# marcin119a/vae-los-angeles

Measured on AMD Instinct MI355X. Metric: training samples/sec, MultiModalVAE batch 65536, higher is better.
Workload: dtype bf16

## Files before the change

### include/mmvae_hip.h

```cpp
#ifndef MMVAE_HIP_H
#define MMVAE_HIP_H
#include <stdint.h>

#ifdef __cplusplus
extern "C" {
#endif

#define MMVAE_OK 0
#define MMVAE_ERR_ARG (-1)
#define MMVAE_ERR_DTYPE (-2)

enum { MMVAE_F32 = 0, MMVAE_BF16 = 1 };
enum { MMVAE_PREC_F32 = 0, MMVAE_PREC_BF16 = 1 };
enum { MMVAE_PRO_NONE = 0, MMVAE_PRO_BN_RELU_DROP = 1, MMVAE_PRO_BN_BWD_APPLY = 2 };
enum { MMVAE_EPI_STORE = 0, MMVAE_EPI_RELU_MASK = 1, MMVAE_EPI_BN_BWD = 2, MMVAE_EPI_LOSS_MSE = 3, MMVAE_EPI_LOSS_BCE_LOGIT = 4 };
enum { MMVAE_ACT_NONE = 0, MMVAE_ACT_RELU = 1, MMVAE_ACT_SIGMOID = 2 };

#define MMVAE_TILE 128

int mmvae_abi_version(void);
int mmvae_set_tuning(int32_t key, int32_t value);

typedef struct {
    const float* src; void* dst;
// ... 98 lines not shown
    const float* scale; const float* shift;
    const uint8_t* mask; int64_t ld_mask; float inv_keep;
    const void* finalize;
    const void* w; int64_t ldw; const float* bias;
} mmvae_latent_enc;
typedef struct {
    int32_t prec, B, L, n_mod;
    mmvae_latent_enc enc_a, enc_b;
    const float* table; const int64_t* site; int32_t S;
    const float* eps;
    float* mu; float* logvar;
    void* z; int64_t ldz;
    const void* w_stem; int64_t ldw_stem; const float* bias_stem; int32_t N_stem;
    void* h0; int64_t ldh0;
} mmvae_latent_fwd_args;
int mmvae_latent_fwd(const mmvae_latent_fwd_args* args, void* stream);

typedef struct {
    int32_t prec, B, S, L, hidden;
    const void* h0; int64_t ldh0;
    const void* w; int64_t ldw; const void* wt; int64_t ldwt; const float* bias;
    const int64_t* site; const float* class_weights;
    const float* mu; const float* logvar;
    float beta, gamma; const float* beta_gamma_dev;
    double* sums;
    float* g_c; int64_t ld_gc;
    void* d0; int64_t ldd0;
    float* g_mu; float* g_lv;
} mmvae_class_tail_args;
int mmvae_class_tail(const mmvae_class_tail_args* args, void* stream);
int mmvae_class_tail_fits(int32_t prec, int32_t S, int32_t hidden, int32_t L, int64_t ldh0, int64_t ldd0);

typedef struct {
    int32_t B, A, D, S, L;
    const float* recon_a; const void* a; int64_t ld_ra, ld_a;
    const float* recon_b; const void* b; int64_t ld_rb, ld_b;
    const float* logits; int64_t ld_logits; const int64_t* site; const float* class_weights;
    const float* mu; const float* logvar;
    float beta, gamma;
    double* sums;
    void* g_a; int32_t g_a_dtype; int64_t ld_ga;
    void* g_b; int32_t g_b_dtype; int64_t ld_gb; int32_t grad_b_wrt_logit;
    float* g_c; int64_t ld_gc;
    float* g_mu; float* g_lv;
    const float* beta_gamma_dev;
    int32_t a_dtype, b_dtype;
} mmvae_loss_args;
int mmvae_vae_loss(const mmvae_loss_args* args, void* stream);
int mmvae_loss_finalize(const double* sums, float beta, float gamma, const float* beta_gamma_dev, float* out5, void* stream);

int mmvae_sigmoid_bwd(int32_t M, int32_t N, const float* g, int64_t ldg, const float* p, int64_t ldpp,
                      void* out, int32_t out_dtype, int64_t ldo, void* stream);

int mmvae_scale_if_needed(void* x, int32_t dtype, int64_t n, const float* scale_dev, void* stream);
#define MMVAE_SCALE_MAX 8
typedef struct { void* x; int64_t n; int32_t dtype; int32_t pad_; } mmvae_scale_item;
int mmvae_scale_many(const mmvae_scale_item* items_host, int32_t n_items, const float* scale_dev, void* stream);

#define MMVAE_CTR_COPIES 16384
int mmvae_noise(uint8_t* mask, int64_t n_mask, float keep_prob, float* eps, int64_t n_eps, uint64_t seed, uint64_t offset,
                uint64_t* offset_dev, int32_t advance, void* stream);
int mmvae_counter_add(uint64_t* counter_dev, uint64_t inc, void* stream);

#define MMVAE_GATHER_MAX 4
typedef struct { const void* src; void* dst; int64_t src_row_stride; int64_t dst_row_stride; int32_t row_bytes; int32_t pad_; } mmvae_gather_item;
int mmvae_gather_rows(const mmvae_gather_item* items_host, int32_t n_items, const int64_t* idx_dev, int32_t rows,
// ... 118 lines not shown
```

### vae-los-angeles_amd/csrc/common.h

```cpp
#pragma once
#include <hip/hip_runtime.h>
#include <stdint.h>
#include "mmvae_hip.h"

namespace mm {

typedef __bf16 bf16;
typedef __attribute__((ext_vector_type(8))) __bf16 bf16x8;
typedef __attribute__((ext_vector_type(4))) __bf16 bf16x4;
typedef __attribute__((ext_vector_type(2))) __bf16 bf16x2;
typedef __attribute__((ext_vector_type(4))) float f32x4;
typedef __attribute__((ext_vector_type(2))) float f32x2;
typedef __attribute__((ext_vector_type(4))) short s16x4;

constexpr int WAVE = 64;
constexpr int TILE = 128;
constexpr int NTHREADS = 256;
constexpr int ROW_BYTES = 128;
constexpr int NUM_CU = 256;

template <typename CT> struct Mma;

template <> struct Mma<bf16> {
    static constexpr int EPC = 8;
// ... 109 lines not shown
    if (n < 0 || n > STAMP_SLOTS) return MMVAE_ERR_ARG;
    hipError_t e = hipMemcpyFromSymbol(out, sym, n * sizeof(uint64_t));
    if (e != hipSuccess || !reset) return (int)e;
    const uint64_t z[STAMP_SLOTS] = {};
    return (int)hipMemcpyToSymbol(sym, z, sizeof(z));
}
int stamp_read_nt(uint64_t*, int, int);
int stamp_read_nt2(uint64_t*, int, int);
int stamp_read_ntp(uint64_t*, int, int);
int stamp_read_tn(uint64_t*, int, int);
int stamp_read_tnw(uint64_t*, int, int);
#else
#define STAMP_T(x)
#define STAMP_ADD(i, d)
#define STAMP_ONLY(...)
#define UNSTAMPED(...) __VA_ARGS__
#define STAMP_BUFFER(name)
#define STAMP_ENTRY()
#endif


struct Tuning {
    int nt_wide_min_m = NUM_CU * 128;
    int nt2_on = 1;
    long split_bytes = 1L << 32;
    long block_bytes = 1L << 31;
    int tn_wide_on = 1;
    int bnbwd_stream = 1;
    int relu_stream = 1;
    int ntp_on = 1;
    int ntp_min_m = 16384;
    int latent_on = 1;
    int class_tail_on = 1;
};
inline Tuning g_tuning;

constexpr int NOT_TAKEN = 1 << 30;

template <auto Kernel, typename... Args>
inline int launch_lds(dim3 grid, dim3 block, int lds, hipStream_t st, const Args&... args) {
    static bool attr_done = false;
    if (!attr_done) {
        hipError_t e = hipFuncSetAttribute((const void*)Kernel, hipFuncAttributeMaxDynamicSharedMemorySize, lds);
        if (e != hipSuccess) return (int)e;
        attr_done = true;
    }
    hipLaunchKernelGGL(Kernel, grid, block, lds, st, args...);
    return (int)hipGetLastError();
}

inline bool needs_row_blocks(long M, long row_bytes) { return M * row_bytes >= g_tuning.split_bytes; }

template <typename F>
inline int for_row_blocks(long M, long row_bytes, F&& block) {
    long rows = g_tuning.block_bytes / row_bytes;
    if (rows <= 0) return MMVAE_ERR_ARG;
    const long nblk = (M + rows - 1) / rows;
    long even = (M + nblk - 1) / nblk;
    if (even >= 256) even = (even + 255) & ~255L;
    if (even <= rows) rows = even;
    else if (rows >= 256) rows &= ~255L;
    for (long r0 = 0; r0 < M; r0 += rows) {
        const int rc = block(r0, (int)(M - r0 < rows ? M - r0 : rows));
        if (rc) return rc;
    }
    return 0;
// ... 31 lines not shown
```

### vae-los-angeles_amd/csrc/elementwise.hip

```cpp
#include <vector>
#include "common.h"
#include "mmvae_hip.h"
#include "fuse_math.h"
#include "loss_terms.h"

namespace mm {

__global__ __launch_bounds__(256) void prep_weights_kernel(const mmvae_prep_item* __restrict__ items) {
    const mmvae_prep_item it = items[blockIdx.y];
    __shared__ float tile[32][33];
    const int tx = threadIdx.x & 31, ty = threadIdx.x >> 5;
    const int tiles_c = (it.dst_cols + 31) / 32, tiles_r = (it.dst_rows + 31) / 32;
    auto put = [&](int r, int c, float v) {
        if (it.dst_dtype == MMVAE_BF16) ((bf16*)it.dst)[(long)r * it.dst_ld + c] = (bf16)v;
        else ((float*)it.dst)[(long)r * it.dst_ld + c] = v;
    };
    for (int t = blockIdx.x; t < tiles_r * tiles_c; t += gridDim.x) {
        const int tr = t / tiles_c, tc = t - tr * tiles_c;
        if (it.transpose) {
#pragma unroll
            for (int k = 0; k < 4; ++k) {
                const int sr = tc * 32 + ty + 8 * k, sc = tr * 32 + tx;
                tile[ty + 8 * k][tx] = (sr < it.src_rows && sc < it.src_cols) ? it.src[(long)sr * it.src_ld + sc] : 0.f;
            }
// ... 209 lines not shown
    }
}

__global__ __launch_bounds__(256) void fuse_bwd_kernel(mmvae_fuse_bwd_args a, int rows_per_block, int use_lds) {
    extern __shared__ float sT[];
    const int L2 = 2 * a.L;
    if (use_lds) { for (int i = threadIdx.x; i < a.S * L2; i += blockDim.x) sT[i] = 0.f; __syncthreads(); }
    const int b0 = blockIdx.x * rows_per_block, b1 = min(a.B, b0 + rows_per_block);
    float* dtab = a.d_table ? a.d_table + (long)(blockIdx.x % (a.table_copies > 0 ? a.table_copies : 1)) * a.S * L2 : nullptr;
    const float inv_n = 1.f / (float)a.n_mod;
    constexpr int U = 4;
    const long iend = (long)b1 * a.L;
    for (long i0 = (long)b0 * a.L + threadIdx.x; i0 < iend; i0 += (long)U * blockDim.x) {
        float dz[U], gm[U], gl[U], ep[U], lv[U];
        int bb[U], ll[U];
        long sidx[U];
#pragma unroll
        for (int u = 0; u < U; ++u) {
            const long i = min(i0 + (long)u * blockDim.x, iend - 1);
            const int b = (int)(i / a.L), l = (int)(i - (long)b * a.L);
            bb[u] = b; ll[u] = l;
            dz[u] = a.dz[(long)b * a.lddz + l];
            if (a.dz2) dz[u] += a.dz2[(long)b * a.lddz + l];
            if (a.dz3) dz[u] += a.dz3[(long)b * a.lddz + l];
            gm[u] = a.g_mu ? a.g_mu[i] : 0.f; gl[u] = a.g_lv ? a.g_lv[i] : 0.f;
            ep[u] = a.eps[i]; lv[u] = a.logvar[i];
            sidx[u] = a.d_table ? a.site[b] : 0;
            if (sidx[u] < 0 || sidx[u] >= a.S) sidx[u] = -1;
        }
#pragma unroll
        for (int u = 0; u < U; ++u) {
            if (i0 + (long)u * blockDim.x >= iend) break;
            const int b = bb[u], l = ll[u];
            float dmu = gm[u] + dz[u];
            float dlv = gl[u] + dz[u] * ep[u] * expf(0.5f * lv[u]) * 0.5f;
            if (a.n_mod > 1) { dmu *= inv_n; dlv *= inv_n; }
            a.d_heads[(long)b * a.ld_heads + l] = dmu;
            a.d_heads[(long)b * a.ld_heads + a.L + l] = dlv;
            if (a.d_heads_lp) {
                bf16* lp = (bf16*)a.d_heads_lp + (long)b * a.ld_heads_lp;
                lp[l] = (bf16)dmu; lp[a.L + l] = (bf16)dlv;
                if (l == 0) for (int e = 2 * a.L; e < a.ld_heads_lp; ++e) lp[e] = (bf16)0.f;
            }
            if (a.d_table && sidx[u] >= 0) {
                const long sx = sidx[u];
                if (use_lds) { atomicAdd(&sT[sx * L2 + l], dmu); atomicAdd(&sT[sx * L2 + a.L + l], dlv); }
                else { unsafeAtomicAdd(&dtab[sx * L2 + l], dmu); unsafeAtomicAdd(&dtab[sx * L2 + a.L + l], dlv); }
            }
        }
    }
    if (use_lds && a.d_table) {
        __syncthreads();
        for (int i = threadIdx.x; i < a.S * L2; i += blockDim.x) if (sT[i] != 0.f) unsafeAtomicAdd(&dtab[i], sT[i]);
    }
}

template <typename GT, int V>
__device__ __forceinline__ void store_vec(GT* p, const float* v) {
    GT o[V];
#pragma unroll
    for (int e = 0; e < V; ++e) o[e] = from_f32<GT>(v[e]);
    if constexpr (sizeof(GT) * V == 16) *(f32x4*)p = *(f32x4*)o;
    else if constexpr (sizeof(GT) * V == 8) *(f32x2*)p = *(f32x2*)o;
    else if constexpr (sizeof(GT) * V == 4) *(float*)p = *(float*)o;
    else for (int e = 0; e < V; ++e) p[e] = o[e];
}

struct RowWalk {
    unsigned cv, dc, vpr;
// ... 750 lines not shown
```

### vae-los-angeles_amd/csrc/fuse_math.h

```cpp
#pragma once
#include "common.h"

namespace mm {

__device__ __forceinline__ float fuse_reparam_elem(float& mu, float& lv, int n_mod, float inv_n, float eps) {
    if (n_mod > 1) { mu *= inv_n; lv *= inv_n; }
    return mu + eps * expf(0.5f * lv);
}

}
```

### vae-los-angeles_amd/csrc/gemm_nt.hip

```cpp
#include "common.h"
#include "mmvae_hip.h"
#include "gemm_src.h"
#include "gemm_nt_epi.h"
#include "gemm_nt2.h"

namespace mm {

STAMP_BUFFER(nt)

__device__ __forceinline__ int swz(int row, int chunk) { return row * ROW_BYTES + ((chunk ^ (row & 7)) << 4); }

template <int WN> struct NtLds {
    static constexpr int BUF = (TILE + 64 * WN) * ROW_BYTES;
    static constexpr int STAGE = 2 * BUF;
    static constexpr int ECOL = STAGE + 4096 + 4 * 64 * WN * 4;
    static constexpr int TOTAL = ECOL + 8 * 64 * WN * 4;
};

template <typename CT, typename Src, typename Epi, int WN>
__global__ __launch_bounds__(128 * WN, 2)
void gemm_nt_kernel(Src src, const CT* __restrict__ W, long ldw, int M, int N, int K, int gx, int gy, Epi epi)
{
    constexpr int EPC = Mma<CT>::EPC;
    constexpr int BK = ROW_BYTES / (int)sizeof(CT);
// ... 275 lines not shown
        SrcBnReluDrop<CT> s{(const CT*)a->a, a->lda, a->M, a->K, a->pro_scale, a->pro_shift, a->pro_mask, a->ld_pro_mask, a->pro_inv_keep, bn_fin_of(a)};
        return dispatch_epi<CT>(a, s, st);
    }
    if (a->a_dtype == MMVAE_BF16) {
        if constexpr (sizeof(CT) == 2) {
            if (a->lda % 8 || ((uintptr_t)a->a & 15)) return MMVAE_ERR_ARG;
            SrcPlain<CT, bf16, 8> s{(const bf16*)a->a, a->lda, a->M, a->K};
            return dispatch_epi<CT>(a, s, st);
        }
        return MMVAE_ERR_DTYPE;
    }
    return with_src_f32<CT>(a->a, a->lda, a->M, a->K, [&](const auto& s) { return dispatch_epi<CT>(a, s, st); });
}

}

extern "C" int mmvae_set_tuning(int32_t key, int32_t value) {
    mm::Tuning& t = mm::g_tuning;
    switch (key) {
    case 0: t.nt_wide_min_m = value; return 0;
    case 2: t.nt2_on = value; return 0;
    case 3:
        if (value != 0 && (value < 17 || value > 32)) return MMVAE_ERR_ARG;
        t.split_bytes = value ? 1L << value : mm::Tuning{}.split_bytes;
        t.block_bytes = t.split_bytes / 2;
        return 0;
    case 4: t.tn_wide_on = value; return 0;
    case 6: t.bnbwd_stream = value; return 0;
    case 7: t.relu_stream = value; return 0;
    case 8: t.ntp_on = value; return 0;
    case 9: t.ntp_min_m = value; return 0;
    case 10: t.latent_on = value; return 0;
    case 12: t.class_tail_on = value; return 0;
    }
    return MMVAE_ERR_ARG;
}

extern "C" int mmvae_gemm_nt(const mmvae_gemm_nt_args* a, void* stream) {
    if (!a || !a->a || !a->w || (!a->c && !(a->epilogue == MMVAE_EPI_BN_BWD && a->bn_phase == 0))) return MMVAE_ERR_ARG;
    if (a->M <= 0 || a->N <= 0 || a->K <= 0) return MMVAE_ERR_ARG;
    if (a->ldw % 64 || ((uintptr_t)a->w & 15)) return MMVAE_ERR_ARG;
    const long lim = 1L << 32;
    if (((long)a->N + 256) * a->ldw * 4 >= lim) return MMVAE_ERR_ARG;
    const long a_row = (long)a->lda * (a->a_dtype == MMVAE_BF16 ? 2 : 4);
    long row_bytes = a_row > (long)a->ld_pro_mask ? a_row : (long)a->ld_pro_mask;
    if (!mm::bn_fin_ok(a)) return MMVAE_ERR_ARG;
    if (mm::needs_row_blocks(a->M, row_bytes)) {
        if (a->pro_finalize || a->pro_out) return MMVAE_ERR_ARG;
        const bool loss_epi = a->epilogue == MMVAE_EPI_LOSS_MSE || a->epilogue == MMVAE_EPI_LOSS_BCE_LOGIT;
        const long hsz = loss_epi ? (a->h_dtype == MMVAE_BF16 ? 2 : 4) : (a->prec == MMVAE_PREC_BF16 ? 2 : 4);
        return mm::for_row_blocks(a->M, row_bytes, [&](long r0, int rows) {
            mmvae_gemm_nt_args s = *a;
            s.M = rows;
            s.a = (const char*)a->a + r0 * a_row;
            if (a->c) s.c = (char*)a->c + r0 * a->ldc * (a->c_dtype == MMVAE_BF16 ? 2 : 4);
            if (a->h) s.h = (const char*)a->h + r0 * a->ldh * hsz;
            if (a->pro_mask) s.pro_mask = a->pro_mask + r0 * a->ld_pro_mask;
            if (a->epi_mask) s.epi_mask = a->epi_mask + r0 * a->ld_epi_mask;
            return mmvae_gemm_nt(&s, stream);
        });
    }
    hipStream_t st = (hipStream_t)stream;
    { const int rc = mm::ntp_dispatch(a, st); if (rc != mm::NOT_TAKEN) return rc; }
    if (a->pro_out) return MMVAE_ERR_ARG;
    if (a->prec == MMVAE_PREC_BF16) return mm::dispatch_src<mm::bf16>(a, st);
    if (a->prec == MMVAE_PREC_F32) return mm::dispatch_src<float>(a, st);
// ... 5 lines not shown
```

### vae-los-angeles_amd/mmvae/_lib.py

```python
import ctypes as C
import os

_HERE = os.path.dirname(os.path.abspath(__file__))
LIB_PATH = os.environ.get("MMVAE_LIB_PATH") or os.path.join(_HERE, "libmmvae_hip.so")
ABI_VERSION = 20

F32, BF16 = 0, 1
PREC_F32, PREC_BF16 = 0, 1
PRO_NONE, PRO_BN_RELU_DROP, PRO_BN_BWD_APPLY = 0, 1, 2
TABLE_COPIES = 8
EPI_STORE, EPI_RELU_MASK, EPI_BN_BWD, EPI_LOSS_MSE, EPI_LOSS_BCE_LOGIT = 0, 1, 2, 3, 4
ACT_NONE, ACT_RELU, ACT_SIGMOID = 0, 1, 2
TILE = 128
TN_GROUP_MAX = 8
KNN_MAXK = 96
SIL_MAXC = 64
PCA_MAXK = 64
LN_MAXN = 1024
WCE_MAXC = 64
CTR_COPIES = 16384

i32, i64, f32, vp = C.c_int32, C.c_int64, C.c_float, C.c_void_p


# ... 52 lines not shown
                ("heads_a", vp), ("heads_b", vp), ("ld_heads", i64),
                ("table", vp), ("site", vp), ("S", i32),
                ("eps", vp), ("mu", vp), ("logvar", vp),
                ("z", vp), ("z_dtype", i32), ("ldz", i64)]


class LatentEnc(C.Structure):
    _fields_ = [("y", vp), ("ldy", i64), ("K", i32), ("scale", vp), ("shift", vp),
                ("mask", vp), ("ld_mask", i64), ("inv_keep", f32), ("finalize", vp),
                ("w", vp), ("ldw", i64), ("bias", vp)]


class LatentFwdArgs(C.Structure):
    _fields_ = [("prec", i32), ("B", i32), ("L", i32), ("n_mod", i32),
                ("enc_a", LatentEnc), ("enc_b", LatentEnc),
                ("table", vp), ("site", vp), ("S", i32),
                ("eps", vp), ("mu", vp), ("logvar", vp),
                ("z", vp), ("ldz", i64),
                ("w_stem", vp), ("ldw_stem", i64), ("bias_stem", vp), ("N_stem", i32),
                ("h0", vp), ("ldh0", i64)]


class ClassTailArgs(C.Structure):
    _fields_ = [("prec", i32), ("B", i32), ("S", i32), ("L", i32), ("hidden", i32),
                ("h0", vp), ("ldh0", i64),
                ("w", vp), ("ldw", i64), ("wt", vp), ("ldwt", i64), ("bias", vp),
                ("site", vp), ("class_weights", vp),
                ("mu", vp), ("logvar", vp),
                ("beta", f32), ("gamma", f32), ("beta_gamma_dev", vp),
                ("sums", vp),
                ("g_c", vp), ("ld_gc", i64),
                ("d0", vp), ("ldd0", i64),
                ("g_mu", vp), ("g_lv", vp)]


class FuseBwdArgs(C.Structure):
    _fields_ = [("B", i32), ("L", i32), ("n_mod", i32),
                ("g_mu", vp), ("g_lv", vp), ("dz", vp), ("dz2", vp), ("dz3", vp), ("lddz", i64),
                ("eps", vp), ("logvar", vp),
                ("d_heads", vp), ("ld_heads", i64),
                ("d_table", vp), ("site", vp), ("S", i32), ("d_heads_lp", vp), ("ld_heads_lp", i64), ("table_copies", i32)]


class LossArgs(C.Structure):
    _fields_ = [("B", i32), ("A", i32), ("D", i32), ("S", i32), ("L", i32),
                ("recon_a", vp), ("a", vp), ("ld_ra", i64), ("ld_a", i64),
                ("recon_b", vp), ("b", vp), ("ld_rb", i64), ("ld_b", i64),
                ("logits", vp), ("ld_logits", i64), ("site", vp), ("class_weights", vp),
                ("mu", vp), ("logvar", vp),
                ("beta", f32), ("gamma", f32),
                ("sums", vp),
                ("g_a", vp), ("g_a_dtype", i32), ("ld_ga", i64),
                ("g_b", vp), ("g_b_dtype", i32), ("ld_gb", i64), ("grad_b_wrt_logit", i32),
                ("g_c", vp), ("ld_gc", i64),
                ("g_mu", vp), ("g_lv", vp), ("beta_gamma_dev", vp), ("a_dtype", i32), ("b_dtype", i32)]


class MetricsArgs(C.Structure):
    _fields_ = [("M", i32), ("N", i32),
                ("pred", vp), ("pred_dtype", i32), ("ld_pred", i64),
                ("target", vp), ("target_dtype", i32), ("ld_target", i64),
                ("col_shift", vp), ("col_acc", vp), ("row_pearson", vp), ("row_cosine", vp)]


class KnnArgs(C.Structure):
    _fields_ = [("q", vp), ("t", vp), ("shift", vp), ("idx", vp), ("dist2", vp), ("work", vp),
# ... 52 lines not shown

class WceArgs(C.Structure):
    _fields_ = [("logits", vp), ("labels", vp), ("class_weights", vp), ("sums", vp), ("g", vp), ("pred", vp), ("nll", vp), ("confusion", vp),
                ("ld", i64), ("ldg", i64),
                ("M", i32), ("C", i32)]


class GatherItem(C.Structure):
    _fields_ = [("src", vp), ("dst", vp), ("src_row_stride", i64), ("dst_row_stride", i64), ("row_bytes", i32), ("pad_", i32)]


class AdamWItem(C.Structure):
    _fields_ = [("p", vp), ("g", vp), ("m", vp), ("v", vp), ("n", i64)]


_SIGNATURES = {
    "mmvae_set_tuning": [i32, i32],
    "mmvae_prep_weights": [vp, i32, vp],
    "mmvae_gemm_nt": [C.POINTER(GemmNtArgs), vp],
    "mmvae_gemm_tn": [C.POINTER(GemmTnArgs), vp],
    "mmvae_gemm_tn_group": [vp, i32, vp],
    "mmvae_bn_finalize": [C.POINTER(BnFinalizeArgs), vp],
    "mmvae_bn_eval_coeffs": [i32, vp, vp, vp, vp, f32, vp, vp, vp, vp, vp],
    "mmvae_bn_bwd_finalize": [C.POINTER(BnBwdFinalizeArgs), vp],
    "mmvae_bn_bwd_apply": [i32, i32, i32, vp, i64, vp, i64, vp, vp, vp, vp],
    "mmvae_bn_bwd_finalize_apply": [i32, i32, i32, vp, i64, vp, i64, vp, vp, vp, vp, vp, vp, vp, i32, vp],
    "mmvae_embed_table_fwd": [i32, i32, i32, vp, vp, vp, vp, vp, vp, vp],
    "mmvae_embed_table_bwd": [i32, i32, i32, vp, vp, vp, vp, i32, vp, vp, vp, vp, vp, vp],
    "mmvae_fuse_reparam_fwd": [C.POINTER(FuseFwdArgs), vp],
    "mmvae_fuse_reparam_bwd": [C.POINTER(FuseBwdArgs), vp],
    "mmvae_latent_fwd": [C.POINTER(LatentFwdArgs), vp],
    "mmvae_class_tail": [C.POINTER(ClassTailArgs), vp],
    "mmvae_class_tail_fits": [i32, i32, i32, i32, i64, i64],
    "mmvae_vae_loss": [C.POINTER(LossArgs), vp],
    "mmvae_loss_finalize": [vp, f32, f32, vp, vp, vp],
    "mmvae_recon_metrics": [C.POINTER(MetricsArgs), vp],
    "mmvae_knn_search": [C.POINTER(KnnArgs), vp],
    "mmvae_knn_work_bytes": [i32, i32, i32, C.POINTER(i64)],
    "mmvae_knn_splits": [i32, i32, C.POINTER(i32), C.POINTER(i32)],
    "mmvae_knn_mean_rows": [vp, i64, vp, i32, i64, vp, i64, i32, i32, i32, i32, vp],
    "mmvae_silhouette_samples": [C.POINTER(SilhouetteArgs), vp],
    "mmvae_silhouette_work_bytes": [i32, i32, i32, C.POINTER(i64)],
    "mmvae_silhouette_splits": [i32, i32, i32, C.POINTER(i32)],
    "mmvae_pca_scatter": [C.POINTER(PcaScatterArgs), vp],
    "mmvae_pca_scatter_splits": [i32, i32, i32, C.POINTER(i32)],
    "mmvae_pca_scatter_work_bytes": [i32, i32, i32, C.POINTER(i64)],
    "mmvae_pca_project": [C.POINTER(PcaProjectArgs), vp],
    "mmvae_tsne_affinities": [C.POINTER(TsneAffinitiesArgs), vp],
    "mmvae_tsne_gradient": [C.POINTER(TsneGradientArgs), vp],
    "mmvae_tsne_gradient_splits": [i32, i32, C.POINTER(i32)],
    "mmvae_tsne_gradient_work_bytes": [i32, i32, C.POINTER(i64)],
    "mmvae_tsne_update": [C.POINTER(TsneUpdateArgs), vp],
    "mmvae_tsne_update_work_bytes": [i32, C.POINTER(i64)],
    "mmvae_ln_act_fwd": [C.POINTER(LnActFwdArgs), vp],
    "mmvae_ln_act_bwd": [C.POINTER(LnActBwdArgs), vp],
    "mmvae_ln_act_bwd_work_bytes": [i32, i32, i32, C.POINTER(i64)],
    "mmvae_wce_mean": [C.POINTER(WceArgs), vp],
    "mmvae_gather_rows": [vp, i32, vp, i32, i64, vp],
    "mmvae_rows_to_bf16": [vp, i32, i64, vp, i64, i32, i32, vp],
    "mmvae_sigmoid_bwd": [i32, i32, vp, i64, vp, i64, vp, i32, i64, vp],
    "mmvae_scale_if_needed": [vp, i32, i64, vp, vp],
    "mmvae_scale_many": [C.POINTER(ScaleItem), i32, vp, vp],
    "mmvae_noise": [vp, i64, f32, vp, i64, C.c_uint64, C.c_uint64, vp, i32, vp],
    "mmvae_counter_add": [vp, C.c_uint64, vp],
    "mmvae_adamw_step": [vp, i32, f32, f32, f32, f32, f32, f32, f32, i32, vp, i32, vp, vp],
    "mmvae_adam_step": [vp, i32, f32, f32, f32, f32, f32, f32, f32, i32, vp, i32, vp, vp],
# ... 42 lines not shown
```

### vae-los-angeles_amd/mmvae/engine.py

```python
import os
from dataclasses import dataclass
from typing import NamedTuple, Optional

import torch

from . import ops
from . import _lib as L_
from .ops import (PREC_BF16, PREC_F32, ACT_NONE, ACT_RELU, ACT_SIGMOID, EPI_RELU_MASK, EPI_BN_BWD, DROP_P,
                  ceil_to, act_dtype, Prologue, BnBwdEpilogue, BnBwdFinalize, BnBwdApply)

_PRECISIONS = {"bf16": PREC_BF16, "fp32": PREC_F32, "f32": PREC_F32}
_default_precision = _PRECISIONS[os.environ.get("MMVAE_PRECISION", "bf16").lower()]
_TINY_DW_MAX = 16384


def set_default_precision(name):
    global _default_precision
    _default_precision = _PRECISIONS[name.lower()]


def default_precision():
    return _default_precision


# ... 596 lines not shown
        slab = torch.empty(min(64 * big, 1 << 25), dtype=torch.float32, device=dev)

        tiny = []

        def tn(prec_, p, q, dw, db, N, K, q_prologue=None, p_prologue=None, tag=None):
            if p_prologue is None and N * K <= _TINY_DW_MAX:
                tiny.append(dict(p=p, q=q, dw=dw, db=db, N=N, K=K, q_prologue=q_prologue))
                return
            ops.gemm_tn(prec_, p, q, dw, db, N, K, q_prologue=q_prologue, p_prologue=p_prologue, slab=slab, tag=tag)

        def flush_tiny(tag):
            if tiny:
                need = ops.TN_GROUP_SPLITS * sum(t_["N"] * t_["K"] for t_ in tiny)
                ops.gemm_tn_group(prec, tiny, torch.empty(need, dtype=torch.float32, device=dev), tag=tag)
                tiny.clear()
        stem = self.dec_stem if all(g is not None for g in g_outs) else None
        D0, off = None, 0
        tail = state.class_tail
        if stem is not None:
            D0 = tail.d0 if tail is not None else torch.empty(B, stem.N, dtype=act_dtype(prec), device=dev)
        for i, (dec, (acts, out), g, is_logit) in enumerate(zip(self.decoders, state.dec, g_outs, g_logit_flags)):
            n0 = dec.linears[0].out_features if stem is not None else 0
            if g is None:
                off += n0
                continue
            dx_done = tail.d0_slice if (tail is not None and tail.index == i and tail.done) else None
            if stem is not None:
                dec.backward(prec, acts, out, g, is_logit, None, grads, tn, d0_out=D0[:, off:off + n0], dx_done=dx_done)
                off += n0
                continue
            dz = torch.empty(B, Ld, dtype=torch.float32, device=dev)
            dec.backward(prec, acts, out, g, is_logit, dz, grads, tn, dx_done=dx_done)
            dzs.append(dz)
        if stem is not None:
            dz = torch.empty(B, Ld, dtype=torch.float32, device=dev)
            ops.gemm_nt(prec, D0, stem.wt, stem.K, stem.N, dz, tag="Decoders.L0.dX")
            dzs.append(dz)
        if not dzs:
            dzs.append(torch.zeros(B, Ld, dtype=torch.float32, device=dev))
        if self.grad_sync is not None:
            self.grad_sync.early(flat, self.early_cut())
        d_heads = torch.empty(B, 2 * Ld, dtype=torch.float32, device=dev)
        d_heads_lp = torch.empty(B, ceil_to(2 * Ld, 8), dtype=torch.bfloat16, device=dev) if prec == PREC_BF16 else None
        ops.fuse_reparam_bwd(B, Ld, state.n_mod, g_mu, g_lv, dzs, state.eps, state.logvar, d_heads, zeros.d_table, site, d_heads_lp=d_heads_lp)
        if state.enc_a is not None:
            self.enc_a.backward(prec, state.enc_a, d_heads, grads, tn, zeros.bwd_stats[:n_a], train=state.train, d_heads_lp=d_heads_lp)
        if state.enc_b is not None:
            self.enc_b.backward(prec, state.enc_b, d_heads, grads, tn, zeros.bwd_stats[n_a:], train=state.train, d_heads_lp=d_heads_lp)
        if site is not None:
            self.enc_c.backward(zeros.d_table, grads)
        flush_tiny("tiny_dW.heads")
        if self.grad_sync is not None:
            self.grad_sync.final(flat)
        return flat, grads
```

### vae-los-angeles_amd/mmvae/ops.py

```python
import ctypes as C
from collections import namedtuple

import torch

from . import _lib as L
from ._lib import (F32, BF16, PREC_F32, PREC_BF16, PRO_NONE, PRO_BN_RELU_DROP, PRO_BN_BWD_APPLY, EPI_STORE, EPI_RELU_MASK,
                   EPI_BN_BWD, EPI_LOSS_MSE, EPI_LOSS_BCE_LOGIT, ACT_NONE, ACT_RELU, ACT_SIGMOID, TILE)

DROP_P = 0.1
BN_EPS, BN_MOMENTUM = 1e-5, 0.1


class KernelProbe:

    def __init__(self, only=None):
        self.records = {}
        self.only = only

    def wants(self, tag):
        return tag is not None and (self.only is None or tag in self.only)

    def begin(self):
        ev = torch.cuda.Event(enable_timing=True)
        ev.record(torch.cuda.current_stream())
# ... 411 lines not shown
    for e, enc in ((a.enc_a, enc_a), (a.enc_b, enc_b)):
        if enc is not None:
            _latent_enc(e, enc)
            nbytes += enc.heads.K * (enc.y.element_size() + (enc.prologue[2] is not None))
    if table is not None:
        a.table, a.site, a.S = table.data_ptr(), _p(site), table.shape[0]
    a.eps, a.mu, a.logvar = eps.data_ptr(), mu.data_ptr(), logvar.data_ptr()
    a.z, a.ldz = z.data_ptr(), _ld(z)
    a.w_stem, a.ldw_stem, a.bias_stem, a.N_stem = stem.w.data_ptr(), stem.w.stride(0), _p(stem.bias), stem.N
    a.h0, a.ldh0 = h0.data_ptr(), _ld(h0)
    return a, B * nbytes


def latent_fwd(prec, B, Ld, enc_a, enc_b, table, site, eps, mu, logvar, z, stem, h0):
    for t in (eps, mu, logvar):
        if tuple(t.shape) != (B, Ld) or not t.is_contiguous():
            raise ValueError(f"latent_fwd: eps / mu / logvar must be contiguous ({B}, {Ld}), got {tuple(t.shape)} / {t.stride()}")
    a, nbytes = latent_fwd_args(prec, B, Ld, enc_a, enc_b, table, site, eps, mu, logvar, z, stem, h0)
    with stream_span("latent.fwd", nbytes):
        L.check(L.load().mmvae_latent_fwd(C.byref(a), _stream()), "mmvae_latent_fwd")


def fuse_reparam_bwd(B, Ld, n_mod, g_mu, g_lv, dzs, eps, logvar, d_heads, d_table, site, d_heads_lp=None):
    dzs = list(dzs) + [None] * (3 - len(dzs))
    copies = d_table.shape[0] if (d_table is not None and d_table.dim() == 3) else 1
    a = L.FuseBwdArgs(B, Ld, n_mod, _p(g_mu), _p(g_lv), dzs[0].data_ptr(), _p(dzs[1]), _p(dzs[2]), _ld(dzs[0]), eps.data_ptr(), logvar.data_ptr(),
                      d_heads.data_ptr(), _ld(d_heads), _p(d_table), _p(site), d_table.shape[-2] if d_table is not None else 0,
                      _p(d_heads_lp), _ld(d_heads_lp) if d_heads_lp is not None else 0, copies)
    n_dz = sum(1 for d in dzs if d is not None)
    with stream_span("fuse_reparam_bwd", B * Ld * 4 * (n_dz + (g_mu is not None) + (g_lv is not None) + 2 + 2)):
        L.check(L.load().mmvae_fuse_reparam_bwd(C.byref(a), _stream()), "mmvae_fuse_reparam_bwd")


def loss_workspace(device):
    buf = torch.zeros(5 * 8 + 5 * 4 + 4, dtype=torch.uint8, device=device)
    return buf[:40].view(torch.float64), buf[40:60].view(torch.float32)


def vae_loss(B, *, recon_a=None, a=None, recon_b=None, b=None, logits=None, site=None, class_weights=None,
             mu=None, logvar=None, beta=1e-3, gamma=1.0, sums=None, g_a=None, g_b=None, grad_b_wrt_logit=False,
             g_c=None, g_mu=None, g_lv=None, beta_gamma_dev=None):
    x = L.LossArgs()
    x.B = B
    if recon_a is not None:
        x.A, x.recon_a, x.a, x.ld_ra, x.ld_a, x.a_dtype = recon_a.shape[1], recon_a.data_ptr(), a.data_ptr(), _ld(recon_a), _ld(a), _dt(a)
    if recon_b is not None:
        x.D, x.recon_b, x.b, x.ld_rb, x.ld_b, x.b_dtype = recon_b.shape[1], recon_b.data_ptr(), b.data_ptr(), _ld(recon_b), _ld(b), _dt(b)
    if logits is not None:
        x.S, x.logits, x.ld_logits, x.site, x.class_weights = logits.shape[1], logits.data_ptr(), _ld(logits), site.data_ptr(), _p(class_weights)
    if mu is not None:
        x.L, x.mu, x.logvar = mu.shape[1], mu.data_ptr(), logvar.data_ptr()
    x.beta, x.gamma, x.sums = beta, gamma, sums.data_ptr()
    if g_a is not None:
        x.g_a, x.g_a_dtype, x.ld_ga = g_a.data_ptr(), _dt(g_a), _ld(g_a)
    if g_b is not None:
        x.g_b, x.g_b_dtype, x.ld_gb, x.grad_b_wrt_logit = g_b.data_ptr(), _dt(g_b), _ld(g_b), int(grad_b_wrt_logit)
    if g_c is not None:
        x.g_c, x.ld_gc = g_c.data_ptr(), _ld(g_c)
    x.g_mu, x.g_lv = _p(g_mu), _p(g_lv)
    x.beta_gamma_dev = _p(beta_gamma_dev)
    assert sums.dtype == torch.float64 and sums.numel() >= 5

    def nbytes():
        n = 0
        for pred, tgt, g in ((recon_a, a, g_a), (recon_b, b, g_b), (logits, None, g_c)):
            if pred is not None:
# ... 539 lines not shown
```

Baseline: 53.65 million.

## Fuse stem dX GEMM with reparameterization backward in one persistent kernel

Result: no change. 54.12 million, median of 6 (+0.9%).

```diff
diff --git a/include/mmvae_hip.h b/include/mmvae_hip.h
--- a/include/mmvae_hip.h
+++ b/include/mmvae_hip.h
@@ -154,6 +154,19 @@
 int mmvae_class_tail_fits(int32_t prec, int32_t S, int32_t hidden, int32_t L, int64_t ldh0, int64_t ldd0);
 
 typedef struct {
+    int32_t prec, B, L, n_mod;
+    const void* d0; int64_t ldd0; int32_t N_stem;
+    const void* wt; int64_t ldwt;
+    const float* g_mu; const float* g_lv;
+    const float* eps; const float* logvar;
+    float* d_heads; int64_t ld_heads;
+    void* d_heads_lp; int64_t ld_heads_lp;
+    float* d_table; const int64_t* site; int32_t S; int32_t table_copies;
+} mmvae_stem_bwd_args;
+int mmvae_stem_bwd(const mmvae_stem_bwd_args* args, void* stream);
+int mmvae_stem_bwd_fits(int32_t prec, int32_t L, int32_t N_stem, int64_t ldd0, int32_t S);
+
+typedef struct {
     int32_t B, A, D, S, L;
     const float* recon_a; const void* a; int64_t ld_ra, ld_a;
     const float* recon_b; const void* b; int64_t ld_rb, ld_b;
diff --git a/vae-los-angeles_amd/csrc/common.h b/vae-los-angeles_amd/csrc/common.h
--- a/vae-los-angeles_amd/csrc/common.h
+++ b/vae-los-angeles_amd/csrc/common.h
@@ -165,6 +165,7 @@
     int ntp_min_m = 16384;
     int latent_on = 1;
     int class_tail_on = 1;
+    int stem_bwd_on = 1;
 };
 inline Tuning g_tuning;
 
diff --git a/vae-los-angeles_amd/csrc/elementwise.hip b/vae-los-angeles_amd/csrc/elementwise.hip
--- a/vae-los-angeles_amd/csrc/elementwise.hip
+++ b/vae-los-angeles_amd/csrc/elementwise.hip
@@ -265,9 +265,8 @@
         for (int u = 0; u < U; ++u) {
             if (i0 + (long)u * blockDim.x >= iend) break;
             const int b = bb[u], l = ll[u];
-            float dmu = gm[u] + dz[u];
-            float dlv = gl[u] + dz[u] * ep[u] * expf(0.5f * lv[u]) * 0.5f;
-            if (a.n_mod > 1) { dmu *= inv_n; dlv *= inv_n; }
+            float dmu, dlv;
+            fuse_reparam_bwd_elem(dz[u], gm[u], gl[u], ep[u], lv[u], a.n_mod, inv_n, dmu, dlv);
             a.d_heads[(long)b * a.ld_heads + l] = dmu;
             a.d_heads[(long)b * a.ld_heads + a.L + l] = dlv;
             if (a.d_heads_lp) {
diff --git a/vae-los-angeles_amd/csrc/fuse_math.h b/vae-los-angeles_amd/csrc/fuse_math.h
--- a/vae-los-angeles_amd/csrc/fuse_math.h
+++ b/vae-los-angeles_amd/csrc/fuse_math.h
@@ -8,4 +8,11 @@
     return mu + eps * expf(0.5f * lv);
 }
 
+__device__ __forceinline__ void fuse_reparam_bwd_elem(float dz, float g_mu, float g_lv, float eps, float lv, int n_mod, float inv_n,
+                                                      float& dmu, float& dlv) {
+    dmu = g_mu + dz;
+    dlv = g_lv + dz * eps * expf(0.5f * lv) * 0.5f;
+    if (n_mod > 1) { dmu *= inv_n; dlv *= inv_n; }
 }
+
+}
diff --git a/vae-los-angeles_amd/csrc/gemm_nt.hip b/vae-los-angeles_amd/csrc/gemm_nt.hip
--- a/vae-los-angeles_amd/csrc/gemm_nt.hip
+++ b/vae-los-angeles_amd/csrc/gemm_nt.hip
@@ -331,6 +331,7 @@
     case 9: t.ntp_min_m = value; return 0;
     case 10: t.latent_on = value; return 0;
     case 12: t.class_tail_on = value; return 0;
+    case 13: t.stem_bwd_on = value; return 0;
     }
     return MMVAE_ERR_ARG;
 }
diff --git a/vae-los-angeles_amd/csrc/stem_bwd.hip b/vae-los-angeles_amd/csrc/stem_bwd.hip
--- /dev/null
+++ b/vae-los-angeles_amd/csrc/stem_bwd.hip
@@ -0,0 +1,239 @@
+#include "common.h"
+#include "mmvae_hip.h"
+#include "fuse_math.h"
+#include "wave_slab.h"
+
+namespace mm {
+
+constexpr int SB_WAVES = 8, SB_THREADS = 64 * SB_WAVES;
+constexpr int SB_NK = 14;
+constexpr int SB_LN = 32;
+constexpr int SB_HN = 48;
+constexpr int SB_FU = SB_HN / 2 * 16 / 64;
+constexpr int SB_HP = SB_HN / 4 * 16 / 64;
+constexpr int SB_MAXTAB = 1024;
+constexpr int SB_WROW = SB_NK * 64 + 16;
+constexpr int SB_DZLD = SB_LN + 4;
+constexpr int SB_HLD = SB_HN + 4;
+constexpr int SB_LPROW = 2 * SB_HN + 16;
+constexpr int SB_OFF_TAB = SB_LN * SB_WROW;
+constexpr int SB_OFF_SCR = SB_OFF_TAB + SB_MAXTAB * 4;
+constexpr int SB_SCR_H = 16 * SB_DZLD * 4;
+constexpr int SB_SCR_LP = SB_SCR_H + 16 * SB_HLD * 4;
+constexpr int SB_SCR_SITE = SB_SCR_LP + 16 * SB_LPROW;
+constexpr int SB_SCR = SB_SCR_SITE + 64;
+constexpr int SB_ST = 2, SB_CT = SB_HN / 16;
+constexpr int SB_LDS = SB_OFF_SCR + SB_WAVES * SB_SCR;
+static_assert(SB_OFF_SCR % 16 == 0 && SB_SCR % 16 == 0 && SB_SCR_H % 16 == 0 && SB_SCR_LP % 16 == 0, "16-byte LDS vectors");
+
+struct SbArgs {
+    int B, L, n_mod, S, ns, nk, nslabs, copies;
+    const bf16* d0; long ldd0; const bf16* wt; long ldwt;
+    const float* g_mu; const float* g_lv; const float* eps; const float* lv;
+    float* dh; long lddh; bf16* lp; long ldlp;
+    float* d_table; const long long* site;
+    int mtile;
+    int dh_vec;
+};
+
+__global__ __launch_bounds__(SB_THREADS) void stem_bwd_kernel(const SbArgs a) {
+    extern __shared__ __attribute__((aligned(16))) unsigned char smem[];
+    const int tid = threadIdx.x, lane = tid & 63, wid = tid >> 6;
+    const int li = lane & 15, lg = lane >> 4;
+    float* const stab = (float*)(smem + SB_OFF_TAB);
+    unsigned char* const scr = smem + SB_OFF_SCR + wid * SB_SCR;
+    float* const sdz = (float*)scr;
+    float* const sh = (float*)(scr + SB_SCR_H);
+    unsigned char* const slp = scr + SB_SCR_LP;
+    int* const ssite = (int*)(scr + SB_SCR_SITE);
+    const int L = a.L, L2 = 2 * a.L;
+    const bool has_tab = a.d_table != nullptr;
+
+    int fr[SB_FU], fl[SB_FU], hr[SB_HP], hc[SB_HP];
+#pragma unroll
+    for (int i = 0; i < SB_FU; ++i) { const int x = lane + 64 * i; fr[i] = x / L; fl[i] = x - fr[i] * L; }
+    const int hppr = L2 >> 2;
+#pragma unroll
+    for (int i = 0; i < SB_HP; ++i) { const int x = lane + 64 * i; hr[i] = x / max(hppr, 1); hc[i] = x - hr[i] * hppr; }
+    const int lppr = (int)(a.ldlp >> 3);
+    const float inv_n = 1.f / (float)a.n_mod;
+    const int total = a.B * L;
+    const int kmax = a.ns - 8;
+
+    bf16x8 raw[SB_NK];
+    float eps_r[SB_FU], lv_r[SB_FU], gm_r[SB_FU] = {}, gl_r[SB_FU] = {};
+    long long site_r = 0;
+    auto fetch = [&](int slab) __attribute__((always_inline)) {
+        const bf16* rowp = a.d0 + (unsigned)min(slab * 16 + li, a.B - 1) * (unsigned)a.ldd0;
+#pragma unroll
+        for (int j = 0; j < SB_NK; ++j)
+            if (j < a.nk) raw[j] = *(const bf16x8*)(rowp + min(32 * j + 8 * lg, kmax));
+#pragma unroll
+        for (int i = 0; i < SB_FU; ++i) {
+            const int idx = min(slab * 16 * L + lane + 64 * i, total - 1);
+            eps_r[i] = a.eps[idx]; lv_r[i] = a.lv[idx];
+        }
+        if (a.g_mu) {
+#pragma unroll
+            for (int i = 0; i < SB_FU; ++i) gm_r[i] = a.g_mu[min(slab * 16 * L + lane + 64 * i, total - 1)];
+        }
+        if (a.g_lv) {
+#pragma unroll
+            for (int i = 0; i < SB_FU; ++i) gl_r[i] = a.g_lv[min(slab * 16 * L + lane + 64 * i, total - 1)];
+        }
+        if (has_tab) site_r = a.site[min(slab * 16 + li, a.B - 1)];
+    };
+
+    const int nw = gridDim.x * SB_WAVES;
+    int slab = blockIdx.x * SB_WAVES + wid;
+    if (slab < a.nslabs) fetch(slab);
+
+    stage_rows<SB_THREADS>(smem, SB_WROW, a.wt, a.ldwt, SB_LN, a.nk * 4, tid, [](int x) { return x; });
+    if (has_tab) for (int i = tid; i < a.S * L2; i += SB_THREADS) stab[i] = 0.f;
+    for (int i = lane; i < (16 * SB_HLD * 4 + 16 * SB_LPROW) / 16; i += 64) ((uint4*)sh)[i] = uint4{0u, 0u, 0u, 0u};
+    f32x4 tacc[SB_ST][SB_CT];
+#pragma unroll
+    for (int m = 0; m < SB_ST; ++m)
+#pragma unroll
+        for (int n = 0; n < SB_CT; ++n) tacc[m][n] = f32x4{0.f, 0.f, 0.f, 0.f};
+    __syncthreads();
+
+    for (; slab < a.nslabs; slab += nw) {
+        f32x4 acc[2] = {f32x4{0.f, 0.f, 0.f, 0.f}, f32x4{0.f, 0.f, 0.f, 0.f}};
+#pragma unroll
+        for (int j = 0; j < SB_NK; ++j) {
+            if (j < a.nk)
+#pragma unroll
+            for (int n = 0; n < 2; ++n) {
+                const bf16x8 wf = *(const bf16x8*)(smem + (16 * n + li) * SB_WROW + (4 * j + lg) * 16);
+                Mma<bf16>::mma(acc[n], wf, raw[j]);
+            }
+        }
+#pragma unroll
+        for (int n = 0; n < 2; ++n) *(f32x4*)(sdz + li * SB_DZLD + 16 * n + 4 * lg) = acc[n];
+        float ep[SB_FU], lv[SB_FU], gm[SB_FU], gl[SB_FU];
+#pragma unroll
+        for (int i = 0; i < SB_FU; ++i) { ep[i] = eps_r[i]; lv[i] = lv_r[i]; gm[i] = gm_r[i]; gl[i] = gl_r[i]; }
+        if (has_tab && lane < 16) ssite[lane] = (slab * 16 + lane < a.B && site_r >= 0 && site_r < a.S) ? (int)site_r : -1;
+        if (slab + nw < a.nslabs) fetch(slab + nw);
+        wave_lds_sync();
+
+#pragma unroll
+        for (int i = 0; i < SB_FU; ++i) {
+            if (lane + 64 * i >= 16 * L) break;
+            const int r = fr[i], l = fl[i];
+            float dmu, dlv;
+            fuse_reparam_bwd_elem(sdz[r * SB_DZLD + l], gm[i], gl[i], ep[i], lv[i], a.n_mod, inv_n, dmu, dlv);
+            sh[r * SB_HLD + l] = dmu; sh[r * SB_HLD + L + l] = dlv;
+            ((bf16*)slp)[r * (SB_LPROW / 2) + l] = (bf16)dmu; ((bf16*)slp)[r * (SB_LPROW / 2) + L + l] = (bf16)dlv;
+            if (has_tab && a.mtile == 0) {
+                const int sx = ssite[r];
+                if (sx >= 0) { atomicAdd(&stab[sx * L2 + l], dmu); atomicAdd(&stab[sx * L2 + L + l], dlv); }
+            }
+        }
+        wave_lds_sync();
+
+        if (a.dh_vec) {
+#pragma unroll
+            for (int i = 0; i < SB_HP; ++i) {
+                if (lane + 64 * i >= 16 * hppr) break;
+                const int row = slab * 16 + hr[i];
+                if (row < a.B) *(f32x4*)(a.dh + (unsigned)row * (unsigned)a.lddh + 4 * hc[i]) = *(const f32x4*)(sh + hr[i] * SB_HLD + 4 * hc[i]);
+            }
+        } else {
+            for (int x = lane; x < 16 * L2; x += 64) {
+                const int r = x / L2, c = x - r * L2, row = slab * 16 + r;
+                if (row < a.B) a.dh[(unsigned)row * (unsigned)a.lddh + c] = sh[r * SB_HLD + c];
+            }
+        }
+        if (a.lp) {
+            for (int x = lane; x < 16 * lppr; x += 64) {
+                const int r = x / lppr, c = x - r * lppr, row = slab * 16 + r;
+                const uint4 v = 8 * c < SB_HN ? *(const uint4*)(slp + r * SB_LPROW + c * 16) : uint4{0u, 0u, 0u, 0u};
+                if (row < a.B) *(uint4*)(a.lp + (unsigned)row * (unsigned)a.ldlp + 8 * c) = v;
+            }
+        }
+        if (a.mtile) {
+#pragma unroll
+            for (int s = 0; s < 4; ++s) {
+                const int k = 4 * s + lg, sx = ssite[k];
+                float bv[SB_CT];
+#pragma unroll
+                for (int n = 0; n < SB_CT; ++n) bv[n] = sx >= 0 ? sh[k * SB_HLD + 16 * n + li] : 0.f;
+#pragma unroll
+                for (int m = 0; m < SB_ST; ++m) {
+                    if (m < a.mtile) {
+                        const float av = sx == 16 * m + li ? 1.f : 0.f;
+#pragma unroll
+                        for (int n = 0; n < SB_CT; ++n)
+                            if (16 * n < L2) tacc[m][n] = __builtin_amdgcn_mfma_f32_16x16x4f32(av, bv[n], tacc[m][n], 0, 0, 0);
+                    }
+                }
+            }
+        }
+
+        wave_lds_sync();
+    }
+
+    if (has_tab) {
+        static_assert(SB_ST * SB_CT * 4 * 64 * 4 <= SB_SCR, "the wave's tiles fit its scratch");
+        if (a.mtile) {
+#pragma unroll
+            for (int m = 0; m < SB_ST; ++m)
+#pragma unroll
+                for (int n = 0; n < SB_CT; ++n)
+#pragma unroll
+                    for (int v = 0; v < 4; ++v) ((float*)scr)[((m * SB_CT + n) * 4 + v) * 64 + lane] = tacc[m][n][v];
+        }
+        __syncthreads();
+        float* const dtab = a.d_table + (long)(blockIdx.x % a.copies) * a.S * L2;
+        for (int i = tid; i < a.S * L2; i += SB_THREADS) {
+            float t = stab[i];
+            if (a.mtile) {
+                const int sx = i / L2, c = i - sx * L2;
+                const int at = (((sx >> 4) * SB_CT + (c >> 4)) * 4 + (sx & 3)) * 64 + ((sx >> 2) & 3) * 16 + (c & 15);
+#pragma unroll
+                for (int w = 0; w < SB_WAVES; ++w) t += ((const float*)(smem + SB_OFF_SCR + w * SB_SCR))[at];
+            }
+            if (t != 0.f) unsafeAtomicAdd(&dtab[i], t);
+        }
+    }
+}
+
+}
+
+extern "C" int mmvae_stem_bwd_fits(int32_t prec, int32_t L, int32_t N_stem, int64_t ldd0, int32_t S) {
+    using namespace mm;
+    if (!g_tuning.stem_bwd_on) return MMVAE_ERR_ARG;
+    if (prec != MMVAE_PREC_BF16) return MMVAE_ERR_ARG;
+    if (L < 1 || 2 * L > SB_HN) return MMVAE_ERR_ARG;
+    if (N_stem < 16 || N_stem % 16 || N_stem > 32 * SB_NK) return MMVAE_ERR_ARG;
+    if (ldd0 % 8 || ldd0 < N_stem) return MMVAE_ERR_ARG;
+    if (S < 0 || (long)S * 2 * L > SB_MAXTAB) return MMVAE_ERR_ARG;
+    return 0;
+}
+
+extern "C" int mmvae_stem_bwd(const mmvae_stem_bwd_args* a, void* stream) {
+    using namespace mm;
+    if (!a) return MMVAE_ERR_ARG;
+    { const int rc = mmvae_stem_bwd_fits(a->prec, a->L, a->N_stem, a->ldd0, a->d_table ? a->S : 0); if (rc) return rc; }
+    if (a->B <= 0 || a->n_mod <= 0 || (long)a->B * a->L >= (1L << 31)) return MMVAE_ERR_ARG;
+    if (!a->d0 || !a->wt || !a->eps || !a->logvar || !a->d_heads) return MMVAE_ERR_ARG;
+    if (a->d_table && (!a->site || a->S <= 0)) return MMVAE_ERR_ARG;
+    if (((uintptr_t)a->d0 & 15) || ((uintptr_t)a->wt & 15) || a->ldwt % 8 || a->ldwt < (a->N_stem + 31) / 32 * 32) return MMVAE_ERR_ARG;
+    if (a->ld_heads < 2 * a->L) return MMVAE_ERR_ARG;
+    if (a->d_heads_lp && (a->ld_heads_lp % 8 || a->ld_heads_lp < 2 * a->L || ((uintptr_t)a->d_heads_lp & 15))) return MMVAE_ERR_ARG;
+    const long lim = 1L << 32;
+    if ((long)a->B * a->ldd0 * 2 >= lim || (long)a->B * a->ld_heads * 4 >= lim || (a->d_heads_lp && (long)a->B * a->ld_heads_lp * 2 >= lim))
+        return MMVAE_ERR_ARG;
+    SbArgs k{};
+    k.B = a->B; k.L = a->L; k.n_mod = a->n_mod; k.S = a->d_table ? a->S : 0; k.ns = a->N_stem; k.nk = (a->N_stem + 31) / 32;
+    k.nslabs = (a->B + 15) / 16; k.copies = a->table_copies > 0 ? a->table_copies : 1;
+    k.d0 = (const bf16*)a->d0; k.ldd0 = a->ldd0; k.wt = (const bf16*)a->wt; k.ldwt = a->ldwt;
+    k.g_mu = a->g_mu; k.g_lv = a->g_lv; k.eps = a->eps; k.lv = a->logvar;
+    k.dh = a->d_heads; k.lddh = a->ld_heads; k.lp = (bf16*)a->d_heads_lp; k.ldlp = a->d_heads_lp ? a->ld_heads_lp : 8;
+    k.d_table = a->d_table; k.site = (const long long*)a->site;
+    k.mtile = (k.S > 0 && k.S <= 16 * SB_ST) ? (k.S + 15) / 16 : 0;
+    k.dh_vec = (2 * a->L) % 4 == 0 && a->ld_heads % 4 == 0 && ((uintptr_t)a->d_heads & 15) == 0;
+    return launch_lds<stem_bwd_kernel>(dim3(persistent_grid(k.nslabs, SB_WAVES)), dim3(SB_THREADS), SB_LDS, (hipStream_t)stream, k);
+}
diff --git a/vae-los-angeles_amd/mmvae/_lib.py b/vae-los-angeles_amd/mmvae/_lib.py
--- a/vae-los-angeles_amd/mmvae/_lib.py
+++ b/vae-los-angeles_amd/mmvae/_lib.py
@@ -108,6 +108,16 @@
                 ("g_c", vp), ("ld_gc", i64),
                 ("d0", vp), ("ldd0", i64),
                 ("g_mu", vp), ("g_lv", vp)]
+
+
+class StemBwdArgs(C.Structure):
+    _fields_ = [("prec", i32), ("B", i32), ("L", i32), ("n_mod", i32),
+                ("d0", vp), ("ldd0", i64), ("N_stem", i32),
+                ("wt", vp), ("ldwt", i64),
+                ("g_mu", vp), ("g_lv", vp), ("eps", vp), ("logvar", vp),
+                ("d_heads", vp), ("ld_heads", i64),
+                ("d_heads_lp", vp), ("ld_heads_lp", i64),
+                ("d_table", vp), ("site", vp), ("S", i32), ("table_copies", i32)]
 
 
 class FuseBwdArgs(C.Structure):
@@ -226,6 +236,8 @@
     "mmvae_latent_fwd": [C.POINTER(LatentFwdArgs), vp],
     "mmvae_class_tail": [C.POINTER(ClassTailArgs), vp],
     "mmvae_class_tail_fits": [i32, i32, i32, i32, i64, i64],
+    "mmvae_stem_bwd": [C.POINTER(StemBwdArgs), vp],
+    "mmvae_stem_bwd_fits": [i32, i32, i32, i64, i32],
     "mmvae_vae_loss": [C.POINTER(LossArgs), vp],
     "mmvae_loss_finalize": [vp, f32, f32, vp, vp, vp],
     "mmvae_recon_metrics": [C.POINTER(MetricsArgs), vp],
diff --git a/vae-los-angeles_amd/mmvae/engine.py b/vae-los-angeles_amd/mmvae/engine.py
--- a/vae-los-angeles_amd/mmvae/engine.py
+++ b/vae-los-angeles_amd/mmvae/engine.py
@@ -652,17 +652,27 @@
             dz = torch.empty(B, Ld, dtype=torch.float32, device=dev)
             dec.backward(prec, acts, out, g, is_logit, dz, grads, tn, dx_done=dx_done)
             dzs.append(dz)
-        if stem is not None:
+        def stem_dx():
             dz = torch.empty(B, Ld, dtype=torch.float32, device=dev)
             ops.gemm_nt(prec, D0, stem.wt, stem.K, stem.N, dz, tag="Decoders.L0.dX")
             dzs.append(dz)
-        if not dzs:
+        fuse_stem = stem is not None and ops.stem_bwd_fits(prec, Ld, stem.N, D0.stride(0), zeros.d_table.shape[-2] if site is not None else 0)
+        if stem is not None and not fuse_stem:
+            stem_dx()
+        if not dzs and not fuse_stem:
             dzs.append(torch.zeros(B, Ld, dtype=torch.float32, device=dev))
         if self.grad_sync is not None:
             self.grad_sync.early(flat, self.early_cut())
         d_heads = torch.empty(B, 2 * Ld, dtype=torch.float32, device=dev)
         d_heads_lp = torch.empty(B, ceil_to(2 * Ld, 8), dtype=torch.bfloat16, device=dev) if prec == PREC_BF16 else None
-        ops.fuse_reparam_bwd(B, Ld, state.n_mod, g_mu, g_lv, dzs, state.eps, state.logvar, d_heads, zeros.d_table, site, d_heads_lp=d_heads_lp)
+        if fuse_stem:
+            try:
+                ops.stem_bwd(prec, B, Ld, state.n_mod, D0, stem, g_mu, g_lv, state.eps, state.logvar, d_heads, zeros.d_table, site, d_heads_lp=d_heads_lp)
+            except L_.MMVAEArgError:
+                fuse_stem = False
+                stem_dx()
+        if not fuse_stem:
+            ops.fuse_reparam_bwd(B, Ld, state.n_mod, g_mu, g_lv, dzs, state.eps, state.logvar, d_heads, zeros.d_table, site, d_heads_lp=d_heads_lp)
         if state.enc_a is not None:
             self.enc_a.backward(prec, state.enc_a, d_heads, grads, tn, zeros.bwd_stats[:n_a], train=state.train, d_heads_lp=d_heads_lp)
         if state.enc_b is not None:
diff --git a/vae-los-angeles_amd/mmvae/ops.py b/vae-los-angeles_amd/mmvae/ops.py
--- a/vae-los-angeles_amd/mmvae/ops.py
+++ b/vae-los-angeles_amd/mmvae/ops.py
@@ -467,6 +467,36 @@
         L.check(L.load().mmvae_fuse_reparam_bwd(C.byref(a), _stream()), "mmvae_fuse_reparam_bwd")
 
 
+def stem_bwd_fits(prec, Ld, n_stem, ldd0, S=0):
+    return L.load().mmvae_stem_bwd_fits(prec, Ld, n_stem, ldd0, S) == 0
+
+
+def stem_bwd_args(prec, B, Ld, n_mod, d0, stem, g_mu, g_lv, eps, logvar, d_heads, d_table, site, d_heads_lp=None):
+    a = L.StemBwdArgs()
+    a.prec, a.B, a.L, a.n_mod = prec, B, Ld, n_mod
+    a.d0, a.ldd0, a.N_stem = _mat(d0, "d0").data_ptr(), _ld(d0), stem.N
+    a.wt, a.ldwt = stem.wt.data_ptr(), stem.wt.stride(0)
+    a.g_mu, a.g_lv, a.eps, a.logvar = _p(g_mu), _p(g_lv), eps.data_ptr(), logvar.data_ptr()
+    a.d_heads, a.ld_heads = d_heads.data_ptr(), _ld(d_heads)
+    if d_heads_lp is not None:
+        a.d_heads_lp, a.ld_heads_lp = d_heads_lp.data_ptr(), _ld(d_heads_lp)
+    if d_table is not None:
+        a.d_table, a.site, a.S = d_table.data_ptr(), _p(site), d_table.shape[-2]
+        a.table_copies = d_table.shape[0] if d_table.dim() == 3 else 1
+    nbytes = B * (d0.element_size() * stem.N + 4 * Ld * (2 + (g_mu is not None) + (g_lv is not None) + 2)
+                  + (2 * _ld(d_heads_lp) if d_heads_lp is not None else 0) + 8 * (d_table is not None))
+    return a, nbytes
+
+
+def stem_bwd(prec, B, Ld, n_mod, d0, stem, g_mu, g_lv, eps, logvar, d_heads, d_table, site, d_heads_lp=None):
+    for t in (g_mu, g_lv, eps, logvar):
+        if t is not None and (tuple(t.shape) != (B, Ld) or not t.is_contiguous() or t.dtype != torch.float32):
+            raise ValueError(f"stem_bwd: g_mu / g_lv / eps / logvar must be contiguous fp32 ({B}, {Ld}), got {tuple(t.shape)} / {t.stride()}")
+    a, nbytes = stem_bwd_args(prec, B, Ld, n_mod, d0, stem, g_mu, g_lv, eps, logvar, d_heads, d_table, site, d_heads_lp)
+    with stream_span("stem.bwd", nbytes):
+        L.check(L.load().mmvae_stem_bwd(C.byref(a), _stream()), "mmvae_stem_bwd")
+
+
 def loss_workspace(device):
     buf = torch.zeros(5 * 8 + 5 * 4 + 4, dtype=torch.uint8, device=device)
     return buf[:40].view(torch.float64), buf[40:60].view(torch.float32)
```
